# danpovey/quantization

Hardware: AMD Instinct MI355X
Metric: vectors encoded/sec at dim=512, 8 codebooks; uint8 codes bit-exact vs ref (higher is better)
Workload: dtype f32 (products: exact 30-bit fixed point on the i8 MFMA); 1 GPU; Quantizer.encode, dim=512, bytes_per_frame=8, codebook_size=256, refine_indexes_iters=5, batch=65536 fp32 Gaussian vectors per GPU (BASELINE.json configs[1]), seeded synthetic codebooks; global_batch=65536, parallelism=batch-sharded x1, no collective

## Files before the change

quantization_amd/csrc/mcq_fix_kernels.h:

```cpp
#pragma once
#include "mcq_kernels.h"

namespace mcq {

typedef int i32x4 __attribute__((ext_vector_type(4)));
typedef int i32x16 __attribute__((ext_vector_type(16)));

constexpr int kFixTile = 128;
constexpr int kFixColPad = 128;
constexpr int kFixRing = 4;
constexpr int kFixSlot = 32768;
constexpr int kFixOperand = 16384;
constexpr int kFixInfo = kFixRing * kFixSlot;
constexpr int kFixLds = kFixInfo + 4096;
constexpr int kFixLdsScreen = kFixLds + 1024;

__host__ __device__ inline long fix_round_rows(long r) { return (r + kFixTile - 1) / kFixTile * kFixTile; }
__host__ __device__ inline int fix_round_cols(int d) { return (d + kFixColPad - 1) / kFixColPad * kFixColPad; }
__host__ __device__ inline size_t fix_plane_bytes(long R, int D) { return (size_t)fix_round_rows(R) * fix_round_cols(D) * 4; }

__device__ __forceinline__ int fix_q(float v, int e) {
    float s = ldexpf(v, 30 - e);
    s = fminf(fmaxf(s, -1073741824.0f), 1073741824.0f);
    return (int)rintf(s);
}

struct FixRowsArgs {
    const float *src;
    int xh;
    long R, Rp;
    int D;
    long ld;
    int Dq;
    int8_t *planes;
    int *exps;
    float *xx;
    const float *bias_src;
    float *bias_dst;
    const float *sub;
    long sub_per, sub_ld;
    const float *dot_vec;
    float *dot_out;
    unsigned *clear;
};

template <int RW, bool DOT>
__device__ __forceinline__ void fix_rows_body(const FixRowsArgs &a, unsigned bid) {
    const float *__restrict__ src = a.src;
    const int xh = a.xh, D = a.D, Dq = a.Dq;
    const long R = a.R, Rp = a.Rp, ld = a.ld;
    float *__restrict__ xx = a.xx;
    const float *__restrict__ bias_src = a.bias_src;
    float *__restrict__ bias_dst = a.bias_dst;
    const float *__restrict__ sub = a.sub;
    int8_t *__restrict__ planes = a.planes;
    constexpr int RPW = RW / 4;
    __shared__ __attribute__((aligned(16))) unsigned tile[128 * RW * 4];
    __shared__ int es[RW];
    const int tid = threadIdx.x, lane = tid & 63, wave = tid >> 6;
    const long row0 = (long)bid * RW;
    if (bias_src && tid < RW && row0 + tid < R) bias_dst[row0 + tid] = bias_src[row0 + tid];
    if (a.clear && bid == 0 && tid == 0) *a.clear = 0u;
    const _Float16 *srch = reinterpret_cast<const _Float16 *>(src);
    const bool vec_ok = ((ld & 3) == 0) && ((D & 3) == 0) && ((reinterpret_cast<uintptr_t>(src) & (xh ? 7 : 15)) == 0);
    auto load4 = [&](long row, int q) -> f32x4 {
        f32x4 v = {0.f, 0.f, 0.f, 0.f};
        if (row >= R || 4 * q >= D) return v;
        if (vec_ok) return xh ? load_h4(srch + row * ld + 4 * q) : *reinterpret_cast<const f32x4 *>(src + row * ld + 4 * q);
#pragma unroll
        for (int c = 0; c < 4; ++c)
            if (4 * q + c < D) v[c] = xh ? (float)srch[row * ld + 4 * q + c] : src[row * ld + 4 * q + c];
        return v;
    };
    auto vec4 = [&](const float *p, int q) -> f32x4 {
        f32x4 v = {0.f, 0.f, 0.f, 0.f};
        if (4 * q >= D) return v;
        if (((D & 3) == 0) && ((reinterpret_cast<uintptr_t>(p) & 15) == 0)) return *reinterpret_cast<const f32x4 *>(p + 4 * q);
#pragma unroll
        for (int c = 0; c < 4; ++c)
            if (4 * q + c < D) v[c] = p[4 * q + c];
        return v;
    };
    auto sub4 = [&](long row, int q) -> f32x4 {
        if (!sub || row >= R) return f32x4{0.f, 0.f, 0.f, 0.f};
        return vec4(sub + (a.sub_per ? (row / a.sub_per) * a.sub_ld : 0), q);
    };
    int ev = 0;
    if (DOT && a.dot_vec) {
        float mv = 0.f;
        for (int q = lane; q < (D + 3) / 4; q += 64) {
            const f32x4 v = vec4(a.dot_vec, q);
#pragma unroll
            for (int c = 0; c < 4; ++c) mv = fmaxf(mv, fabsf(v[c]));
        }
        for (int s = 32; s >= 1; s >>= 1) mv = fmaxf(mv, __shfl_xor(mv, s, 64));
        const int be = (int)((__float_as_uint(mv) >> 23) & 0xff);
        ev = (be < 1 ? 1 : be) - 126;
    }
    const bool cached = (RW == 4) && D <= 1024;
    f32x4 cache[RW == 4 ? RPW : 1][4];
#pragma unroll
    for (int rr = 0; rr < RPW; ++rr) {
        const long row = row0 + RPW * wave + rr;
        float m = 0.f, pe = 0.f;
        if (cached) {
            f32x4 raw[4], sv4[4];
#pragma unroll
            for (int j = 0; j < 4; ++j) raw[j] = load4(row, lane + 64 * j);
#pragma unroll
            for (int j = 0; j < 4; ++j) sv4[j] = sub4(row, lane + 64 * j);
#pragma unroll
            for (int j = 0; j < 4; ++j) cache[RW == 4 ? rr : 0][j] = sub ? raw[j] - sv4[j] : raw[j];
#pragma unroll
            for (int j = 0; j < 4; ++j)
#pragma unroll
                for (int c = 0; c < 4; ++c) {
                    m = fmaxf(m, fabsf(cache[RW == 4 ? rr : 0][j][c]));
                    pe = fmaf(cache[RW == 4 ? rr : 0][j][c], cache[RW == 4 ? rr : 0][j][c], pe);
                }
        } else {
            for (int q = lane; q < (D + 3) / 4; q += 64) {
                const f32x4 raw = load4(row, q);
                const f32x4 v = sub ? raw - sub4(row, q) : raw;
#pragma unroll
                for (int c = 0; c < 4; ++c) {
                    m = fmaxf(m, fabsf(v[c]));
                    pe = fmaf(v[c], v[c], pe);
                }
            }
        }
        for (int s = 32; s >= 1; s >>= 1) m = fmaxf(m, __shfl_xor(m, s, 64));
        if (xx) pe = wave_sum_butterfly(pe);
        if (lane == 0) {
            const int be = (int)((__float_as_uint(m) >> 23) & 0xff);
            const int e = (be < 1 ? 1 : be) - 126;
            es[RPW * wave + rr] = e;
            if (row < Rp) a.exps[row] = e;
            if (xx && row < R) xx[row] = pe;
        }
    }
    __syncthreads();
    int T[RPW][4];
#pragma unroll
    for (int rr = 0; rr < RPW; ++rr)
#pragma unroll
        for (int i = 0; i < 4; ++i) T[rr][i] = 0;
    auto limbs4 = [&](const f32x4 &v, int e, unsigned (&w)[4]) {
#pragma unroll
        for (int i = 0; i < 4; ++i) w[i] = 0u;
#pragma unroll
        for (int c = 0; c < 4; ++c) {
            int r = fix_q(v[c], e);
#pragma unroll
            for (int i = 3; i >= 1; --i) {
                const int l = (int)(int8_t)(r & 0xff);
                w[i] |= (unsigned)(l & 0xff) << (8 * c);
                r = (r - l) >> 8;
            }
            w[0] |= (unsigned)(r & 0xff) << (8 * c);
        }
    };
    for (int c0 = 0; c0 < Dq; c0 += 512) {
        const int ncol = (Dq - c0 < 512) ? Dq - c0 : 512;
#pragma unroll
        for (int rr = 0; rr < RPW; ++rr) {
            const int rl = RPW * wave + rr;
            const int e = es[rl];
#pragma unroll
            for (int j = 0; j < 2; ++j) {
                const int q = lane + 64 * j;
                if (q >= ncol / 4) continue;
                f32x4 v;
                if (cached) v = cache[RW == 4 ? rr : 0][((c0 >> 9) * 2 + j) & 3];
                else v = sub ? load4(row0 + rl, c0 / 4 + q) - sub4(row0 + rl, c0 / 4 + q) : load4(row0 + rl, c0 / 4 + q);
                unsigned w[4];
                limbs4(v, e, w);
                if (DOT && a.dot_vec) {
                    unsigned mw[4];
                    limbs4(vec4(a.dot_vec, c0 / 4 + q), ev, mw);
#pragma unroll
                    for (int i = 0; i < 4; ++i)
#pragma unroll
                        for (int jj = 0; i + jj < 4; ++jj) T[rr][i + jj] = __builtin_amdgcn_sdot4((int)w[i], (int)mw[jj], T[rr][i + jj], false);
                }
                const int chunk = q >> 2, word = q & 3;
#pragma unroll
                for (int i = 0; i < 4; ++i) tile[((chunk * 4 + i) * RW + rl) * 4 + word] = w[i];
            }
        }
        __syncthreads();
        const int nplanes = ncol / 16 * 4;
        for (int p = tid / RW; p < nplanes; p += 256 / RW) {
            const int rl = tid % RW;
            if (row0 + rl < Rp) {
                const i32x4 v = *reinterpret_cast<const i32x4 *>(&tile[(p * RW + rl) * 4]);
                *reinterpret_cast<i32x4 *>(planes + (((long)(c0 / 16) * 4 + p) * Rp + row0 + rl) * 16) = v;
            }
        }
        __syncthreads();
    }
    if (DOT && a.dot_vec) {
#pragma unroll
        for (int rr = 0; rr < RPW; ++rr) {
            int t4[4];
#pragma unroll
            for (int i = 0; i < 4; ++i) {
                int t = T[rr][i];
                for (int s = 32; s >= 1; s >>= 1) t += __shfl_xor(t, s, 64);
                t4[i] = t;
            }
            const long row = row0 + RPW * wave + rr;
            if (lane == 0 && row < R) {
                float tt = (float)t4[3];
                tt = __builtin_fmaf((float)t4[2], 256.0f, tt);
                tt = __builtin_fmaf((float)t4[1], 65536.0f, tt);
                tt = __builtin_fmaf((float)t4[0], 16777216.0f, tt);
                a.dot_out[row] = ldexpf(tt, es[RPW * wave + rr] + ev - 36);
            }
        }
    }
}

template <int RW>
__global__ void __launch_bounds__(256) k_fix_rows(const FixRowsArgs a) { fix_rows_body<RW, false>(a, blockIdx.x); }

template <int RW>
__global__ void __launch_bounds__(256) k_fix_rows2(const FixRowsArgs a, const FixRowsArgs b, unsigned blocks_a) {
    if (blockIdx.x < blocks_a) fix_rows_body<RW, false>(a, blockIdx.x);
    else fix_rows_body<RW, true>(b, blockIdx.x - blocks_a);
}

enum { FG_STORE = 0, FG_LOGITS = 1, FG_SCREEN = 2 };

struct FixGemm {
    const int8_t *A, *B;
    const int *ea, *eb;
    long RA, RB;
    long M, N;
    int Dq;
    int walk_rows;
    float *out;
    long ldo;
    const float *bias;
    const float *wmu;
    const float *lscale_ptr;
    float lscale;
    float *logits;
    void *idx;
    int idx_wide;
    int K, ncb;
    unsigned *und_cnt, *und_list;
    unsigned und_cap;
};

__device__ __forceinline__ void fg_store_idx(const FixGemm &g, long pos, long entry) {
    if (g.idx_wide) static_cast<uint16_t *>(g.idx)[pos] = (uint16_t)entry;
    else static_cast<uint8_t *>(g.idx)[pos] = (uint8_t)entry;
}

template <int MODE>
__global__ void __launch_bounds__(512)
k_fgemm(const FixGemm g) {
    extern __shared__ __attribute__((aligned(16))) char smem[];
    constexpr bool SCREEN = MODE == FG_SCREEN, LOGITS = MODE != FG_STORE;
    constexpr int NL = SCREEN ? 3 : 4;
    const int tid = threadIdx.x, lane = tid & 63, wave = tid >> 6;
    const int wm = wave & 1, wn = wave >> 1;
    const int r32 = lane & 31, kh = lane >> 5;
    const long MT = g.RA / kFixTile, NT = g.RB / kFixTile;
    const int H = (LOGITS && g.K > kFixTile) ? g.K / kFixTile : 1;
    const long big = g.walk_rows ? NT : MT, small_units = (g.walk_rows ? MT : NT) / H;
    const int xcd = blockIdx.x & 7, slot = blockIdx.x >> 3, per_xcd = gridDim.x >> 3;
    auto tile_of = [&](long t, long &m0, long &n0) -> bool {
        const long unit = t / H, half = t % H;
        const long idx = slot + unit * per_xcd;
        const long bt = (idx / small_units) * 8 + xcd, st = (idx % small_units) * H + half;
        m0 = (g.walk_rows ? st : bt) * kFixTile;
        n0 = (g.walk_rows ? bt : st) * kFixTile;
        return bt < big;
    };
    i32x16 acc[2][NL];
    const int nst = g.Dq / 32;
    const int wu = __builtin_amdgcn_readfirstlane(wave);
    const int op = wu >> 2, chunk = (wu >> 1) & 1, half = wu & 1;
    const long R = op ? g.RB : g.RA;
    const long pl = R * 16, sstride = 8 * R * 16;
    const unsigned dbase = (unsigned)(size_t)smem + op * kFixOperand + (4 * chunk) * 2048 + half * 1024;
    const unsigned voff = lane * 16, voff4 = lane * 4;
    auto base_of = [&](long m0, long n0) { return (op ? g.B + n0 * 16 : g.A + m0 * 16) + (long)(4 * chunk) * R * 16 + half * 1024; };
    auto issue1 = [&](const int8_t *p, int st, int g4) {
        const int8_t *pg = p + g4 * pl;
        const unsigned d = dbase + (st % kFixRing) * kFixSlot + g4 * 2048;
        asm volatile(
            "s_mov_b32 m0, %[d]\n\ts_nop 0\n\t"
            "global_load_lds_dwordx4 %[vo], %[p]\n\t"
            :
            : [vo] "v"(voff), [p] "s"(pg), [d] "s"(d)
            : "memory");
    };
    auto issue_info = [&](long m0, long n0) {
        if (wu < (LOGITS ? 8 : 4)) {
            const void *src = wu < 2 ? static_cast<const void *>(g.ea + m0 + 64 * wu)
                                     : (wu < 4 ? static_cast<const void *>(g.eb + n0 + 64 * (wu - 2))
                                               : (wu < 6 ? static_cast<const void *>(g.bias + m0 + 64 * (wu - 4))
                                                         : static_cast<const void *>(g.wmu + m0 + 64 * (wu - 6))));
            const unsigned d = (unsigned)(size_t)smem + kFixInfo + 256 * (wu < 6 ? wu : wu + 4);
            asm volatile(
                "s_mov_b32 m0, %[d]\n\ts_nop 0\n\t"
                "global_load_lds_dword %[vo], %[p]\n\t"
                :
                : [vo] "v"(voff4), [p] "s"(src), [d] "s"(d)
                : "memory");
        }
    };
    long m0, n0, m0n = 0, n0n = 0;
    if (!tile_of(0, m0, n0)) return;
    const int8_t *pcur = base_of(m0, n0), *pnext = pcur;
    auto step = [&](int st, const i32x4 (&a)[2][NL], const i32x4 (&b)[NL], i32x4 (&an)[2][NL], i32x4 (&bn)[NL]) {
        const char *base = smem + ((st + 1) % kFixRing) * kFixSlot;
        const int8_t *p = (st + 4 < nst) ? pcur + (st + 4) * sstride : pnext + (st + 4 - nst) * sstride;
        constexpr int PI[10] = {0, 0, 1, 0, 1, 2, 0, 1, 2, 3};
        constexpr int PJ[10] = {0, 1, 0, 2, 1, 0, 3, 2, 1, 0};
        constexpr int LO[5] = {0, SCREEN ? 2 : 3, SCREEN ? 4 : 6, SCREEN ? 6 : 8, 10};
#pragma unroll
        for (int g4 = 0; g4 < NL; ++g4) {
            issue1(p, st, g4);
#pragma unroll
            for (int t = 0; t < 2; ++t)
                an[t][g4] = *reinterpret_cast<const i32x4 *>(base + (kh * 4 + g4) * 2048 + (64 * wm + 32 * t + r32) * 16);
            bn[g4] = *reinterpret_cast<const i32x4 *>(base + kFixOperand + (kh * 4 + g4) * 2048 + (32 * wn + r32) * 16);
#pragma unroll
            for (int q = LO[g4]; q < LO[g4 + 1]; ++q)
#pragma unroll
                for (int ta = 0; ta < 2; ++ta)
                    acc[ta][PI[q] + PJ[q]] =
                        __builtin_amdgcn_mfma_i32_32x32x32_i8(a[ta][PI[q]], b[PJ[q]], acc[ta][PI[q] + PJ[q]], 0, 0, 0);
            __builtin_amdgcn_sched_barrier(0);
        }
    };
    i32x4 a0[2][NL], b0[NL], a1[2][NL], b1[NL];
    issue_info(m0, n0);
#pragma unroll
    for (int q = 0; q < 4; ++q)
#pragma unroll
        for (int g4 = 0; g4 < NL; ++g4) issue1(pcur + q * sstride, q, g4);
    if constexpr (SCREEN) asm volatile("s_waitcnt vmcnt(9)" ::: "memory");
    else asm volatile("s_waitcnt vmcnt(12)" ::: "memory");
    __builtin_amdgcn_s_barrier();
#pragma unroll
    for (int l = 0; l < NL; ++l) {
#pragma unroll
        for (int t = 0; t < 2; ++t)
            a0[t][l] = *reinterpret_cast<const i32x4 *>(smem + (kh * 4 + l) * 2048 + (64 * wm + 32 * t + r32) * 16);
        b0[l] = *reinterpret_cast<const i32x4 *>(smem + kFixOperand + (kh * 4 + l) * 2048 + (32 * wn + r32) * 16);
    }
    int *info = reinterpret_cast<int *>(smem + kFixInfo);
    float *infof = reinterpret_cast<float *>(smem + kFixInfo);
    float runv = 0.f;
    int runk = 0;
    float runs = 0.f, runt = 0.f, runq = 0.f;
    int runj = 0, rune = 0;
    for (long t = 0;; ++t) {
        const bool has_next = tile_of(t + 1, m0n, n0n);
        pnext = has_next ? base_of(m0n, n0n) : pcur;
#pragma unroll
        for (int a = 0; a < 2; ++a)
#pragma unroll
            for (int s = 0; s < NL; ++s)
#pragma unroll
                for (int v = 0; v < 16; ++v) acc[a][s][v] = 0;
        for (int st = 0; st < nst; st += 2) {
            if constexpr (SCREEN) asm volatile("s_waitcnt vmcnt(6)\n\ts_waitcnt lgkmcnt(0)" ::: "memory");
            else asm volatile("s_waitcnt vmcnt(8)\n\ts_waitcnt lgkmcnt(0)" ::: "memory");
            __builtin_amdgcn_s_barrier();
            step(st, a0, b0, a1, b1);
            if constexpr (SCREEN) asm volatile("s_waitcnt vmcnt(6)\n\ts_waitcnt lgkmcnt(0)" ::: "memory");
            else asm volatile("s_waitcnt vmcnt(8)\n\ts_waitcnt lgkmcnt(0)" ::: "memory");
            __builtin_amdgcn_s_barrier();
            step(st + 1, a1, b1, a0, b0);
        }
        auto value = [&](int ta, int v, int e) -> float {
            float tt;
            if constexpr (SCREEN) tt = __fmul_rn((float)acc[ta][2][v], 256.0f);
            else tt = __builtin_fmaf((float)acc[ta][2][v], 256.0f, (float)acc[ta][NL - 1][v]);
            tt = __builtin_fmaf((float)acc[ta][1][v], 65536.0f, tt);
            tt = __builtin_fmaf((float)acc[ta][0][v], 16777216.0f, tt);
            return ldexpf(tt, e);
        };
        int rbase = 64 * wm + 4 * kh, cbase = 32 * wn + r32;
        asm volatile("" : "+v"(rbase), "+v"(cbase));
        i32x4 er[2][4];
#pragma unroll
        for (int ta = 0; ta < 2; ++ta)
#pragma unroll
            for (int q = 0; q < 4; ++q) er[ta][q] = *reinterpret_cast<const i32x4 *>(&info[rbase + 32 * ta + 8 * q]);
        const bool full = (m0 + kFixTile <= g.M) && (n0 + kFixTile <= g.N);
        const int ecol = info[128 + cbase] - 36;
        const int rows_left = (int)((g.M - m0 - rbase) > 128 ? 128 : (g.M - m0 - rbase));
        if (MODE == FG_STORE) {
            const bool col_ok = n0 + cbase < g.N;
            float *orow = g.out + (m0 + rbase) * g.ldo + n0 + cbase;
            if (full) {
#pragma unroll
                for (int ta = 0; ta < 2; ++ta)
#pragma unroll
                    for (int v = 0; v < 16; ++v) {
                        const int ro = 32 * ta + 8 * (v >> 2) + (v & 3);
                        orow[(long)ro * g.ldo] = value(ta, v, er[ta][v >> 2][v & 3] + ecol);
                    }
            } else {
#pragma unroll
                for (int ta = 0; ta < 2; ++ta)
#pragma unroll
                    for (int v = 0; v < 16; ++v) {
                        const int ro = 32 * ta + 8 * (v >> 2) + (v & 3);
                        const float val = value(ta, v, er[ta][v >> 2][v & 3] + ecol);
                        if (col_ok && ro < rows_left) orow[(long)ro * g.ldo] = val;
                    }
            }
        } else if constexpr (SCREEN) {
            const float ls = g.lscale_ptr ? *g.lscale_ptr : g.lscale;
            float bv[4], sv[4], tv[4], qm = 0.f;
            int bk[4], sk[4];
            const long col = n0 + cbase;
#pragma unroll
            for (int ta = 0; ta < 2; ++ta) {
#pragma unroll
                for (int v4 = 0; v4 < 4; ++v4) {
                    const f32x4 br4 = *reinterpret_cast<const f32x4 *>(&infof[256 + rbase + 32 * ta + 8 * v4]);
                    const f32x4 wm4 = *reinterpret_cast<const f32x4 *>(&infof[640 + rbase + 32 * ta + 8 * v4]);
#pragma unroll
                    for (int c = 0; c < 4; ++c) {
                        const int v = 4 * v4 + c;
                        const int rl = rbase + 32 * ta + 8 * v4 + c;
                        const float s2 = __fmul_rn(__fadd_rn(value(ta, v, er[ta][v4][c] + ecol), wm4[c]), ls);
                        const float val = __fadd_rn(s2, br4[c]);
                        qm = fmaxf(qm, fmaxf(fabsf(s2), fabsf(val)));
                        const int gi = 2 * ta + (v4 >> 1);
                        if ((v4 & 1) == 0 && c == 0) { bv[gi] = val; bk[gi] = sk[gi] = rl; sv[gi] = tv[gi] = -INFINITY; }
                        else {
                            const bool c1 = val > bv[gi], c2 = val > sv[gi];
                            tv[gi] = __builtin_amdgcn_fmed3f(tv[gi], sv[gi], val);
                            sv[gi] = __builtin_amdgcn_fmed3f(sv[gi], bv[gi], val);
                            sk[gi] = c1 ? bk[gi] : (c2 ? rl : sk[gi]);
                            bk[gi] = c1 ? rl : bk[gi];
                            bv[gi] = fmaxf(bv[gi], val);
                        }
                    }
                }
            }
            int em = info[lane] > info[lane + 64] ? info[lane] : info[lane + 64];
            for (int s = 32; s >= 1; s >>= 1) { const int o = __shfl_xor(em, s, 64); em = o > em ? o : em; }
            auto merge = [](float &b1, int &k1, float &s1, int &j1, float &t1, float b2, int k2, float s2, int j2, float t2) {
                if (b2 > b1) {
                    float f = b1; b1 = b2; b2 = f;
                    f = s1; s1 = s2; s2 = f;
                    t1 = t2;
                    int i = k1; k1 = k2; k2 = i;
                    j1 = j2;
                }
                if (b2 > s1) { t1 = fmaxf(s1, s2); s1 = b2; j1 = k2; }
                else t1 = fmaxf(t1, b2);
            };
            const float cA = 16.5f * 16384.0f * (float)g.Dq;
            auto undecided = [&](float v, float s, float q, int e) {
                const float margin = __fadd_rn(__fadd_rn(__fmul_rn(ldexpf(cA, e + ecol), ls), __fmul_rn(q, 1.9073486328125e-6f)), 7.5231638452626401e-37f);
                return !(__fsub_rn(v, s) > margin);
            };
            auto append = [&](long pos, unsigned second_entry, bool many) {
                const unsigned at = atomicAdd(g.und_cnt, 1u);
                if (at < g.und_cap) {
                    g.und_list[2 * (size_t)at] = (unsigned)pos;
                    g.und_list[2 * (size_t)at + 1] = second_entry | (many ? 0x80000000u : 0u);
                }
            };
            const int K = g.K;
#pragma unroll
            for (int gi = 0; gi < 4; ++gi)
                merge(bv[gi], bk[gi], sv[gi], sk[gi], tv[gi], __shfl_xor(bv[gi], 32, 64), __shfl_xor(bk[gi], 32, 64),
                      __shfl_xor(sv[gi], 32, 64), __shfl_xor(sk[gi], 32, 64), __shfl_xor(tv[gi], 32, 64));
            qm = fmaxf(qm, __shfl_xor(qm, 32, 64));
            if (K >= 32) {
                merge(bv[0], bk[0], sv[0], sk[0], tv[0], bv[1], bk[1], sv[1], sk[1], tv[1]);
                merge(bv[2], bk[2], sv[2], sk[2], tv[2], bv[3], bk[3], sv[3], sk[3], tv[3]);
            }
            if (K >= 64) merge(bv[0], bk[0], sv[0], sk[0], tv[0], bv[2], bk[2], sv[2], sk[2], tv[2]);
            if (K <= 64) {
                if (kh == 0) {
                    const int span = K / 16;
#pragma unroll
                    for (int gi = 0; gi < 4; ++gi) {
                        const long row = m0 + bk[gi];
                        if ((gi % span) == 0 && col < g.N && row < g.M) {
                            fg_store_idx(g, col * g.ncb + row / K, row % K);
                            if (undecided(bv[gi], sv[gi], qm, em))
                                append(col * g.ncb + row / K, (unsigned)((m0 + sk[gi]) % K), undecided(bv[gi], tv[gi], qm, em));
                        }
                    }
                }
            } else {
                float *exv = infof + 384, *exs = infof + 768, *exq = infof + 896;
                int *exk = info + 384 + 128;
                float *ext = reinterpret_cast<float *>(smem + kFixInfo + 4096);
                int *exj = reinterpret_cast<int *>(smem + kFixInfo + 4096 + 512);
                if (wm == 1 && kh == 0) {
                    exv[cbase] = bv[0]; exk[cbase] = bk[0]; exs[cbase] = sv[0]; exq[cbase] = qm;
                    ext[cbase] = tv[0]; exj[cbase] = sk[0];
                }
                asm volatile("s_waitcnt lgkmcnt(0)" ::: "memory");
                __builtin_amdgcn_s_barrier();
                if (wm == 0 && kh == 0) {
                    const int hf = (int)(t % H);
                    float v = bv[0], s = sv[0], t3 = tv[0], q = fmaxf(qm, exq[cbase]);
                    int kk = bk[0], jj = sk[0];
                    merge(v, kk, s, jj, t3, exv[cbase], exk[cbase], exs[cbase], exj[cbase], ext[cbase]);
                    kk += (int)m0;
                    jj += (int)m0;
                    if (hf > 0) {
                        merge(v, kk, s, jj, t3, runv, runk, runs, runj, runt);
                        q = fmaxf(q, runq);
                        em = em > rune ? em : rune;
                    }
                    runv = v; runk = kk; runs = s; runj = jj; runt = t3; runq = q; rune = em;
                    const long k = kk;
                    if (hf == H - 1 && col < g.N && k < g.M) {
                        fg_store_idx(g, col * g.ncb + k / K, k % K);
                        if (undecided(v, s, q, em)) append(col * g.ncb + k / K, (unsigned)(jj % K), undecided(v, t3, q, em));
                    }
                }
            }
        } else {
            const float ls = g.lscale_ptr ? *g.lscale_ptr : g.lscale;
            float bv[4];
            int bk[4];
            const long col = n0 + cbase;
            float *lrow = g.logits ? g.logits + col * g.ldo + m0 + rbase : nullptr;
#pragma unroll
            for (int ta = 0; ta < 2; ++ta) {
#pragma unroll
                for (int v4 = 0; v4 < 4; ++v4) {
                    const f32x4 br4 = *reinterpret_cast<const f32x4 *>(&infof[256 + rbase + 32 * ta + 8 * v4]);
                    const f32x4 wm4 = *reinterpret_cast<const f32x4 *>(&infof[640 + rbase + 32 * ta + 8 * v4]);
                    f32x4 q4;
#pragma unroll
                    for (int c = 0; c < 4; ++c) {
                        const int v = 4 * v4 + c;
                        const int rl = rbase + 32 * ta + 8 * v4 + c;
                        const float val = __fadd_rn(__fmul_rn(__fadd_rn(value(ta, v, er[ta][v4][c] + ecol), wm4[c]), ls), br4[c]);
                        q4[c] = val;
                        const int gi = 2 * ta + (v4 >> 1);
                        if ((v4 & 1) == 0 && c == 0) { bv[gi] = val; bk[gi] = rl; }
                        else if (val > bv[gi]) { bv[gi] = val; bk[gi] = rl; }
                    }
                    if (lrow && (full || (col < g.N && 32 * ta + 8 * v4 < rows_left)))
                        *reinterpret_cast<f32x4 *>(lrow + 32 * ta + 8 * v4) = q4;
                }
            }
            if (g.idx) {
                auto better = [](float v1, int k1, float v2, int k2) { return (v1 > v2) | ((v1 == v2) & (k1 < k2)); };
                const int K = g.K;
#pragma unroll
                for (int gi = 0; gi < 4; ++gi) {
                    const float ov = __shfl_xor(bv[gi], 32, 64);
                    const int ok = __shfl_xor(bk[gi], 32, 64);
                    if (better(ov, ok, bv[gi], bk[gi])) { bv[gi] = ov; bk[gi] = ok; }
                }
                if (K >= 32) {
                    if (bv[1] > bv[0]) { bv[0] = bv[1]; bk[0] = bk[1]; }
                    if (bv[3] > bv[2]) { bv[2] = bv[3]; bk[2] = bk[3]; }
                }
                if (K >= 64 && bv[2] > bv[0]) { bv[0] = bv[2]; bk[0] = bk[2]; }
                if (K <= 64) {
                    if (kh == 0) {
                        const int span = K / 16;
#pragma unroll
                        for (int gi = 0; gi < 4; ++gi) {
                            const long row = m0 + bk[gi];
                            if ((gi % span) == 0 && col < g.N && row < g.M) fg_store_idx(g, col * g.ncb + row / K, row % K);
                        }
                    }
                } else {
                    float *exv = infof + 384;
                    int *exk = info + 384 + 128;
                    if (wm == 1 && kh == 0) { exv[cbase] = bv[0]; exk[cbase] = bk[0]; }
                    asm volatile("s_waitcnt lgkmcnt(0)" ::: "memory");
                    __builtin_amdgcn_s_barrier();
                    if (wm == 0 && kh == 0) {
                        const int hf = (int)(t % H);
                        float v = bv[0];
                        long k = m0 + bk[0];
                        if (better(exv[cbase], exk[cbase], bv[0], bk[0])) { v = exv[cbase]; k = m0 + exk[cbase]; }
                        if (hf > 0 && !(v > runv)) { v = runv; k = runk; }
                        runv = v;
                        runk = (int)k;
                        if (hf == H - 1 && col < g.N && k < g.M) fg_store_idx(g, col * g.ncb + k / K, k % K);
                    }
                }
            }
        }
        if (!has_next) break;
        asm volatile("s_waitcnt lgkmcnt(0)" ::: "memory");
        __builtin_amdgcn_s_barrier();
        m0 = m0n;
        n0 = n0n;
        pcur = pnext;
        issue_info(m0, n0);
    }
    asm volatile("s_waitcnt vmcnt(0)" ::: "memory");
}

struct FixRecheck {
    const int8_t *W, *X;
    const int *ew, *ex;
    long RW, RX;
    int Dq;
    const float *bias, *wmu, *lscale_ptr;
    float lscale;
    void *idx;
    int idx_wide;
    int K, ncb;
    const unsigned *cnt, *list;
    unsigned cap;
};

__global__ void __launch_bounds__(256) k_fscreen_recheck(const FixRecheck a) {
    const int lane = threadIdx.x & 63;
    const unsigned wv = __builtin_amdgcn_readfirstlane(blockIdx.x * 4 + (threadIdx.x >> 6)), nwv = gridDim.x * 4;
    unsigned n = *a.cnt;
    n = n < a.cap ? n : a.cap;
    const float ls = a.lscale_ptr ? *a.lscale_ptr : a.lscale;
    const int K = a.K, nch = a.Dq / 16;
    for (unsigned i = wv; i < n; i += nwv) {
        const unsigned pos = a.list[2 * (size_t)i], snd = a.list[2 * (size_t)i + 1];
        const long col = pos / (unsigned)a.ncb;
        const int cb = (int)(pos % (unsigned)a.ncb);
        const int ecol = a.ex[col] - 36;
        auto chunk = [&](int (&T)[4], int c, long row) {
            i32x4 xl[4], wl[4];
#pragma unroll
            for (int l = 0; l < 4; ++l) {
                xl[l] = *reinterpret_cast<const i32x4 *>(a.X + (((long)c * 4 + l) * a.RX + col) * 16);
                wl[l] = *reinterpret_cast<const i32x4 *>(a.W + (((long)c * 4 + l) * a.RW + row) * 16);
            }
#pragma unroll
            for (int p = 0; p < 4; ++p)
#pragma unroll
                for (int q = 0; p + q < 4; ++q)
#pragma unroll
                    for (int d = 0; d < 4; ++d) T[p + q] = __builtin_amdgcn_sdot4(wl[p][d], xl[q][d], T[p + q], false);
        };
        auto logit = [&](const int (&T)[4], long row) -> float {
            float tt = (float)T[3];
            tt = __builtin_fmaf((float)T[2], 256.0f, tt);
            tt = __builtin_fmaf((float)T[1], 65536.0f, tt);
            tt = __builtin_fmaf((float)T[0], 16777216.0f, tt);
            return __fadd_rn(__fmul_rn(__fadd_rn(ldexpf(tt, a.ew[row] + ecol), a.wmu[row]), ls), a.bias[row]);
        };
        float bv = -INFINITY;
        int bk = 0x7fffffff;
        if ((snd & 0x80000000u) == 0) {
            const int first = a.idx_wide ? (int)static_cast<const uint16_t *>(a.idx)[pos] : (int)static_cast<const uint8_t *>(a.idx)[pos];
            const int j = (lane < 32) ? first : (int)snd;
            const long row = (long)cb * K + j;
            int T[4] = {0, 0, 0, 0};
            for (int c = lane & 31; c < nch; c += 32) chunk(T, c, row);
#pragma unroll
            for (int p = 0; p < 4; ++p)
                for (int sft = 16; sft >= 1; sft >>= 1) T[p] += __shfl_xor(T[p], sft, 64);
            bv = logit(T, row);
            bk = j;
        } else {
            for (int j = lane; j < K; j += 64) {
                const long row = (long)cb * K + j;
                int T[4] = {0, 0, 0, 0};
#pragma unroll 4
                for (int c = 0; c < nch; ++c) chunk(T, c, row);
                const float val = logit(T, row);
                if (j == lane || val > bv) { bv = val; bk = j; }
            }
        }
        for (int s = 32; s >= 1; s >>= 1) {
            const float ov = __shfl_xor(bv, s, 64);
            const int ok = __shfl_xor(bk, s, 64);
            if ((ov > bv) | ((ov == bv) & (ok < bk))) { bv = ov; bk = ok; }
        }
        if (lane == 0) {
            if (a.idx_wide) static_cast<uint16_t *>(a.idx)[pos] = (uint16_t)bk;
            else static_cast<uint8_t *>(a.idx)[pos] = (uint8_t)bk;
        }
    }
}

}
```

Before: 14.68 million vectors/s.

## Split wide recheck entries across the whole block instead of one wave

In the screen-recheck kernel, a block now takes four list entries at a time. Narrow (two-candidate) entries are still handled one per wave. Wide entries, which need a full scan over K codewords, are now spread over all 256 threads of the block, with a cross-wave reduction through shared memory. This is meant to cut the tail latency of full scans, where one wave used to do all K rows alone. The cost is extra block-wide barriers, and waves now wait on each other every iteration.

```diff
diff --git a/quantization_amd/csrc/mcq_fix_kernels.h b/quantization_amd/csrc/mcq_fix_kernels.h
--- a/quantization_amd/csrc/mcq_fix_kernels.h
+++ b/quantization_amd/csrc/mcq_fix_kernels.h
@@ -624,17 +624,24 @@
 };
 
 __global__ void __launch_bounds__(256) k_fscreen_recheck(const FixRecheck a) {
+    __shared__ int wide_of[2][4];
+    __shared__ float part_v[4][4];
+    __shared__ int part_k[4][4];
     const int lane = threadIdx.x & 63;
-    const unsigned wv = __builtin_amdgcn_readfirstlane(blockIdx.x * 4 + (threadIdx.x >> 6)), nwv = gridDim.x * 4;
+    const int w = __builtin_amdgcn_readfirstlane((int)(threadIdx.x >> 6));
+    const unsigned nwv = gridDim.x * 4;
     unsigned n = *a.cnt;
     n = n < a.cap ? n : a.cap;
     const float ls = a.lscale_ptr ? *a.lscale_ptr : a.lscale;
     const int K = a.K, nch = a.Dq / 16;
-    for (unsigned i = wv; i < n; i += nwv) {
-        const unsigned pos = a.list[2 * (size_t)i], snd = a.list[2 * (size_t)i + 1];
-        const long col = pos / (unsigned)a.ncb;
-        const int cb = (int)(pos % (unsigned)a.ncb);
-        const int ecol = a.ex[col] - 36;
+    int par = 0;
+    for (unsigned i0 = blockIdx.x * 4; i0 < n; i0 += nwv, par ^= 1) {
+        const unsigned i = i0 + (unsigned)w;
+        const bool have = i < n;
+        const unsigned pos = have ? a.list[2 * (size_t)i] : 0u, snd = have ? a.list[2 * (size_t)i + 1] : 0u;
+        long col = pos / (unsigned)a.ncb;
+        int cb = (int)(pos % (unsigned)a.ncb);
+        int ecol = a.ex[col] - 36;
         auto chunk = [&](int (&T)[4], int c, long row) {
             i32x4 xl[4], wl[4];
 #pragma unroll
@@ -656,9 +663,20 @@
             tt = __builtin_fmaf((float)T[0], 16777216.0f, tt);
             return __fadd_rn(__fmul_rn(__fadd_rn(ldexpf(tt, a.ew[row] + ecol), a.wmu[row]), ls), a.bias[row]);
         };
-        float bv = -INFINITY;
-        int bk = 0x7fffffff;
-        if ((snd & 0x80000000u) == 0) {
+        auto wave_first_max = [&](float &bv, int &bk) {
+            for (int s = 32; s >= 1; s >>= 1) {
+                const float ov = __shfl_xor(bv, s, 64);
+                const int ok = __shfl_xor(bk, s, 64);
+                if ((ov > bv) | ((ov == bv) & (ok < bk))) { bv = ov; bk = ok; }
+            }
+        };
+        auto store_code = [&](unsigned at, int k) {
+            if (a.idx_wide) static_cast<uint16_t *>(a.idx)[at] = (uint16_t)k;
+            else static_cast<uint8_t *>(a.idx)[at] = (uint8_t)k;
+        };
+        const bool wide = have && (snd & 0x80000000u) != 0;
+        if (lane == 0) wide_of[par][w] = wide ? 1 : 0;
+        if (have && !wide) {
             const int first = a.idx_wide ? (int)static_cast<const uint16_t *>(a.idx)[pos] : (int)static_cast<const uint8_t *>(a.idx)[pos];
             const int j = (lane < 32) ? first : (int)snd;
             const long row = (long)cb * K + j;
@@ -667,26 +685,40 @@
 #pragma unroll
             for (int p = 0; p < 4; ++p)
                 for (int sft = 16; sft >= 1; sft >>= 1) T[p] += __shfl_xor(T[p], sft, 64);
-            bv = logit(T, row);
-            bk = j;
-        } else {
-            for (int j = lane; j < K; j += 64) {
+            float bv = logit(T, row);
+            int bk = j;
+            wave_first_max(bv, bk);
+            if (lane == 0) store_code(pos, bk);
+        }
+        __syncthreads();
+        for (int s = 0; s < 4; ++s) {
+            if (!wide_of[par][s]) continue;
+            const unsigned wpos = a.list[2 * (size_t)(i0 + (unsigned)s)];
+            col = wpos / (unsigned)a.ncb;
+            cb = (int)(wpos % (unsigned)a.ncb);
+            ecol = a.ex[col] - 36;
+            float bv = -INFINITY;
+            int bk = 0x7fffffff;
+            for (int j = (int)threadIdx.x; j < K; j += 256) {
                 const long row = (long)cb * K + j;
                 int T[4] = {0, 0, 0, 0};
 #pragma unroll 4
                 for (int c = 0; c < nch; ++c) chunk(T, c, row);
                 const float val = logit(T, row);
-                if (j == lane || val > bv) { bv = val; bk = j; }
-            }
-        }
-        for (int s = 32; s >= 1; s >>= 1) {
-            const float ov = __shfl_xor(bv, s, 64);
-            const int ok = __shfl_xor(bk, s, 64);
-            if ((ov > bv) | ((ov == bv) & (ok < bk))) { bv = ov; bk = ok; }
-        }
-        if (lane == 0) {
-            if (a.idx_wide) static_cast<uint16_t *>(a.idx)[pos] = (uint16_t)bk;
-            else static_cast<uint8_t *>(a.idx)[pos] = (uint8_t)bk;
+                if (j == (int)threadIdx.x || val > bv) { bv = val; bk = j; }
+            }
+            wave_first_max(bv, bk);
+            if (lane == 0) { part_v[s][w] = bv; part_k[s][w] = bk; }
+            __syncthreads();
+            if (threadIdx.x == 0) {
+#pragma unroll
+                for (int q = 1; q < 4; ++q) {
+                    const float ov = part_v[s][q];
+                    const int ok = part_k[s][q];
+                    if ((ov > bv) | ((ov == bv) & (ok < bk))) { bv = ov; bk = ok; }
+                }
+                store_code(wpos, bk);
+            }
         }
     }
 }
```

Result: no change. 14.62 million vectors/s (-0.4%).
